# haliphinx/TCE-RVOS

Hardware: AMD Instinct MI355X
Metric: clips/s (T=5, 360×640, Swin-T) at 1/2/4/8 MI355X; mask IoU vs ref (higher is better)
Workload: dtype f32 (3xf16-split MFMA, f32 accumulate); 1 GPU; swin_t_p4w7 T=5 360x640 + 32-token text, B=1 clip per forward, flags --with_box_refine --binary --f_token 8 --qtrans (BASELINE config 2); clips_in_flight_per_gpu=1, clips_per_forward=1, same_clip_in_group=False, ranks_per_gpu=1, parallelism=clip-sharded x1

## Files before the change

include/tce_rvos.h:

```cpp
#ifndef TCE_RVOS_H
#define TCE_RVOS_H
#include <stdint.h>

#ifdef __cplusplus
extern "C" {
#endif

typedef void* tceStream;

int tce_abi_version(void);
const char* tce_last_error(void);

typedef struct {
  const float* A;
  const float* A2;
  const float* W;
  const float* bias;
  const float* res;
  float* C;
  int32_t M, N, K;
  int32_t lda, lda2, ldw, ldc, ldres;
  int32_t act, res_mode;
  int32_t batch;
  int64_t sA, sA2, sW, sBias, sC, sRes;
// ... 159 lines not shown
  float* out;
  const float *g_in, *be_in, *g_out, *be_out;
  int64_t ldx, lda2, ldres, ldo;
  int64_t sX, sA2, sRes, sOut;
  int32_t M, N, K, batch, a2_rows, act, res_mode;
  float eps_in, eps_out;
} tceRowLinArgs;
int64_t tce_rowlin_packed_bytes(int32_t N, int32_t K);
int tce_rowlin_pack_f32(const float* W, int64_t ldw, void* packed, int32_t N, int32_t K, tceStream stream);
int tce_rowlin_f32(const tceRowLinArgs* args, tceStream stream);

int64_t tce_conv3x3_packed_bytes(int32_t Cin, int32_t N);
int tce_conv3x3_pack_f32(const float* w, void* packed, int32_t Cin, int32_t N, tceStream stream);
int tce_conv3x3_f32(const float* x, int64_t ldx, const void* packed, const float* bias, float* out, int64_t ldo, int32_t T,
                    int32_t H, int32_t W, int32_t Cin, int32_t N, tceStream stream);

typedef struct {
  const float* x;
  const float* a2;
  const void* packed;
  const float* bo;
  const float* res;
  float* out;
  const float *g_out, *be_out;
  int64_t ldx, lda2, ldres, ldo;
  int64_t sX, sRes, sOut, sW;
  int32_t M, batch, a2_rows, res_mode, group;
  float eps_out;
  int32_t w_div;
} tceXattnArgs;
// ... 63 lines not shown
```

include/tce_rvos_debug.h:

```cpp
#ifndef TCE_RVOS_DEBUG_H
#define TCE_RVOS_DEBUG_H
#include <stdint.h>
#ifdef __cplusplus
extern "C" {
#endif
int tce_gemm_force_tile(int32_t tile);
int tce_debug_set_stamp_buffer(long long* dev_buf);
int tce_debug_set_epilogue(int32_t lds_staged);
int tce_debug_ffn_set_stamp_buffer(long long* dev_buf);
int tce_debug_ffn_set_half(int32_t mode);
int tce_debug_msda_set_lds(int32_t on);
int tce_debug_window_attn_set_mfma(int32_t on);
int tce_debug_mha_set_split(int32_t on);
int tce_debug_msda_set_fewq(int32_t on);
int tce_debug_conv3x3_set_waves(int32_t waves);
#ifdef __cplusplus
}
#endif
#endif
```

tce-rvos_amd/_lib.py:

```python
import ctypes as C
import os

HERE = os.path.dirname(os.path.abspath(__file__))
LIB_PATH = os.environ.get("TCE_LIB") or os.path.join(HERE, "lib", "libtce_rvos.so")

c_f = C.c_void_p
i32, i64, f32 = C.c_int32, C.c_int64, C.c_float


class GemmArgs(C.Structure):
    _fields_ = [("A", c_f), ("A2", c_f), ("W", c_f), ("bias", c_f), ("res", c_f), ("C", c_f),
                ("M", i32), ("N", i32), ("K", i32),
                ("lda", i32), ("lda2", i32), ("ldw", i32), ("ldc", i32), ("ldres", i32),
                ("act", i32), ("res_mode", i32), ("batch", i32),
                ("sA", i64), ("sA2", i64), ("sW", i64), ("sBias", i64), ("sC", i64), ("sRes", i64),
                ("conv", i32), ("T", i32), ("H", i32), ("Wd", i32), ("Cin", i32), ("Ho", i32), ("Wo", i32),
                ("kh", i32), ("kw", i32), ("stride", i32), ("pad", i32)]


class RowLinArgs(C.Structure):
    _fields_ = [("x", c_f), ("a2", c_f), ("packed", c_f), ("bias", c_f), ("res", c_f), ("out", c_f),
                ("g_in", c_f), ("be_in", c_f), ("g_out", c_f), ("be_out", c_f),
                ("ldx", i64), ("lda2", i64), ("ldres", i64), ("ldo", i64),
                ("sX", i64), ("sA2", i64), ("sRes", i64), ("sOut", i64),
# ... 93 lines not shown
    "tce_ffn_fused_split_f32": (i32, [c_f, i64, c_f, c_f, c_f, c_f, f32, c_f, c_f, f32, c_f, i64, i32, i32, i32, i32, c_f, i64, c_f, i32, c_f]),
    "tce_xattn_prepare_f32": (i32, [c_f, c_f, c_f, c_f, c_f, c_f, c_f, i32, i32, i32, c_f]),
    "tce_ffn_pack_batched_f32": (i32, [c_f, c_f, c_f, c_f, i32, i32, i32, c_f]),
    "tce_xattn_fused_f32": (i32, [C.POINTER(XattnArgs), c_f]),
    "tce_xattn_ffn_fused_f32": (i32, [C.POINTER(XattnArgs), C.POINTER(XattnFfnArgs), c_f]),
    "tce_ffn_pack_chain_f32": (i32, [c_f, c_f, c_f, c_f, i32, i32, c_f]),
    "tce_xattn_pack_f32": (i32, [c_f, c_f, c_f, c_f, c_f, i32, i32, i32, c_f]),
    "tce_xattn_prepare_lens_f32": (i32, [c_f, c_f, c_f, c_f, c_f, c_f, c_f, i32, i32, i32, c_f, c_f]),
    "tce_xattn_pack_lens_f32": (i32, [c_f, c_f, c_f, c_f, c_f, i32, i32, i32, c_f, c_f]),
    "tce_rowlin_packed_bytes": (i64, [i32, i32]),
    "tce_rowlin_pack_f32": (i32, [c_f, i64, c_f, i32, i32, c_f]),
    "tce_rowlin_f32": (i32, [C.POINTER(RowLinArgs), c_f]),
    "tce_conv3x3_packed_bytes": (i64, [i32, i32]),
    "tce_conv3x3_pack_f32": (i32, [c_f, c_f, i32, i32, c_f]),
    "tce_conv3x3_f32": (i32, [c_f, i64, c_f, c_f, c_f, i64, i32, i32, i32, i32, i32, c_f]),
    "tce_fewrow_linear_f32": (i32, [C.POINTER(FewRowArgs), c_f]),
    "tce_thin_linear_splits": (i32, [i32, i32, i32]),
    "tce_thin_partials_f32": (i32, [c_f, i64, i32, c_f, i32, c_f, i64, c_f, i32, i32, i32, c_f]),
    "tce_splitk_reduce_f32": (i32, [c_f, i32, i32, i32, c_f, i32, c_f, i32, i32, c_f, i32, c_f, c_f, f32, c_f]),
    "tce_mha_small64_splits_f32": (i32, [c_f, i32, c_f, c_f, i32, i32, f32, c_f]),
    "tce_swin_attn_packed_bytes": (i64, [i32]),
    "tce_swin_attn_pack_f32": (i32, [c_f, c_f, c_f, i32, c_f]),
    "tce_swin_attn_fused_f32": (i32, [c_f, i64, c_f, c_f, c_f, c_f, c_f, c_f, f32, c_f, i64, i32, i32, i32, i32, i32, c_f]),
    "tce_graph_begin": (i32, [c_f]),
    "tce_graph_end": (i32, [c_f, C.POINTER(C.c_void_p)]),
    "tce_graph_launch": (i32, [C.c_void_p, c_f]),
    "tce_graph_destroy": (i32, [C.c_void_p]),
    "tce_graph_group": (i32, [C.POINTER(C.c_void_p), i32, C.POINTER(C.c_void_p)]),
}

DEBUG_SIGNATURES = {
    "tce_gemm_force_tile": (i32, [i32]),
    "tce_debug_set_stamp_buffer": (i32, [c_f]),
    "tce_debug_set_epilogue": (i32, [i32]),
    "tce_debug_ffn_set_stamp_buffer": (i32, [c_f]),
    "tce_debug_ffn_set_half": (i32, [i32]),
    "tce_debug_msda_set_lds": (i32, [i32]),
    "tce_debug_window_attn_set_mfma": (i32, [i32]),
    "tce_debug_mha_set_split": (i32, [i32]),
    "tce_debug_msda_set_fewq": (i32, [i32]),
    "tce_debug_conv3x3_set_waves": (i32, [i32]),
}

_LIB = None


class TceError(RuntimeError):
    pass


def lib():
    global _LIB
    if _LIB is None:
        if not os.path.exists(LIB_PATH):
            raise TceError(f"{LIB_PATH} not found: build the HIP extension first "
                           f"(python -c 'import __graft_entry__ as g; g.build()'); there is no fallback path")
# ... 24 lines not shown
```

tce-rvos_amd/csrc/chain.hip:

```cpp
#include "common.h"
#include "gemm_epilogue.h"
#include "frag.h"
#include "../../include/tce_rvos.h"
#include "../../include/tce_rvos_debug.h"

namespace {

#ifndef FFN_ABL
#define FFN_ABL 0
#endif
static __device__ long long* g_ffn_stamps = nullptr;


template <int K, bool HAS_A2 = true>
__device__ __forceinline__ void load_x_frags(const float* __restrict__ x, const long long ldx,
                                             const float* __restrict__ a2, const long long lda2, const int a2_rows,
                                             const int m0, const int M, float* __restrict__ wt, const int lane,
                                             const float* __restrict__ g_in, const float* __restrict__ be_in,
                                             const float eps, h16x8 (&xh)[K / 16], h16x8 (&xl)[K / 16],
                                             const int single = 0) {
  constexpr int NP = K / 32;
  const int cr = lane >> 3, cp = (lane & 7) * 4;
  const int r = lane & 31, hf = lane >> 5;
  f32x4 v[NP][4];
// ... 834 lines not shown
      return;
    }
  }
  if (a.single) hipLaunchKernelGGL((rowlin_kernel<K, false, true>), grid, block, 0, s, a);
  else hipLaunchKernelGGL((rowlin_kernel<K, false, false>), grid, block, 0, s, a);
}

inline bool ffn_shape_ok(int C, int Hd) { return (C == 96 || C == 128 || C == 192 || C == 256) && Hd > 0 && Hd % 32 == 0; }
inline int ffn_waves(int C) { return C <= 128 ? 8 : 4; }
inline int ffn_pieces(int C) {
  const int w = ffn_waves(C);
  return (1 + 2 * (C / 16) + 4 * (C / 32) + w - 1) / w * w;
}
inline long long ffn_units(int C, int Hd) { return (long long)(Hd / 32 + 2) * ffn_pieces(C) * 64; }

struct FfnSplitPlan {
  int p = 0, k[2] = {0, 0}, nblk = 0;
  long long ws_floats = 0;
};
inline FfnSplitPlan ffn_split_plan(int M, int C, int Hd, int batch) {
  FfnSplitPlan best;
  const int B = tce_cdiv(M, 32 * ffn_waves(C)), NC = Hd / 32, CUS = 256;
  if (C != 256 || NC < 24 || batch < 1) return best;
  const int OVP = 3, OVF = 4;
  auto rounds = [&](long long wgs) { return (double)((wgs + CUS - 1) / CUS); };
  double best_cost = 0.75 * rounds((long long)B * batch) * (NC + 1 + OVP + OVF);
  for (int p = 1; p <= 2; ++p) {
    const int wd = p == 1 ? 0 : (p * NC - 2 * (1 + OVP)) / (p + 1), ws_ = p == 1 ? (NC + 1) / 2 : wd + 1 + OVP;
    int k[2] = {ws_, 0};
    bool ok = ws_ >= 1 && ws_ <= NC - 1;
    for (int i = 1; i < p && ok; ++i) {
      k[i] = wd - (NC - k[i - 1]);
      ok = k[i] >= 1 && k[i] <= NC - 1;
    }
    if (!ok) continue;
    const int busiest = ws_ > NC - k[p - 1] ? ws_ : NC - k[p - 1];
    const double cost = rounds((long long)tce_cdiv(B, p) * (p + 1) * batch) * (busiest + 1 + OVP + OVF);
// ... 11 lines not shown
}

static int g_ffn_half = 0;

template <int C, int WAVES>
void ffn_launch(const FfnArgs& a, int act, hipStream_t s, int batch = 1) {
  if constexpr (C == 256) {
    if (a.sp_p > 0 && act == 1) {
      const dim3 grid(tce_cdiv(a.nblk, a.sp_p) * (a.sp_p + 1), batch), block(64 * WAVES);
      if (a.single) hipLaunchKernelGGL((ffn_fused_kernel<C, WAVES, 1, true, 0, true>), grid, block, 0, s, a);
      else hipLaunchKernelGGL((ffn_fused_kernel<C, WAVES, 1, false, 0, true>), grid, block, 0, s, a);
      return;
    }
  }
  if constexpr (C <= 128 && WAVES == 8) {
    const long long b8 = (long long)tce_cdiv(a.M, 256) * batch, b4 = (long long)tce_cdiv(a.M, 128) * batch;
    const double c8 = (double)((b8 + 255) / 256);
    const long long rem = b4 % 512;
    const double c4 = (double)(b4 / 512) + (rem == 0 ? 0.0 : rem <= 256 ? 0.5 : 1.0);
    if (act == 2 && g_ffn_half >= 0 && (g_ffn_half > 0 || c4 <= c8)) {
      const dim3 grid(tce_cdiv(a.M, 128), batch), block(256);
      if (a.single) hipLaunchKernelGGL((ffn_fused_kernel<C, 4, 2, true>), grid, block, 0, s, a);
      else hipLaunchKernelGGL((ffn_fused_kernel<C, 4, 2, false>), grid, block, 0, s, a);
      return;
    }
  }
  const dim3 grid(tce_cdiv(a.M, 32 * WAVES), batch), block(64 * WAVES);
  if (a.single) {
    if (act == 1) hipLaunchKernelGGL((ffn_fused_kernel<C, WAVES, 1, true>), grid, block, 0, s, a);
    else if (act == 2) hipLaunchKernelGGL((ffn_fused_kernel<C, WAVES, 2, true>), grid, block, 0, s, a);
  } else {
    if (act == 1) hipLaunchKernelGGL((ffn_fused_kernel<C, WAVES, 1, false>), grid, block, 0, s, a);
    else if (act == 2) hipLaunchKernelGGL((ffn_fused_kernel<C, WAVES, 2, false>), grid, block, 0, s, a);
  }
// ... 128 lines not shown
  if (p_lo < P) stage_out[p_lo * 64 + lane] = ol;
}

constexpr int CONV_PAD_STAGES = 6;

struct ConvArgs {
  const float* x;
  const unsigned char* wpk;
  const float* bias;
  float* out;
  long long ldx, ldo;
  int H, W, M;
  int* range_flag;
  int single;
  int m_off;
};

#ifndef CONV_ABL
#define CONV_ABL 0
#endif

template <int BYTE_OFF>
__device__ __forceinline__ void gload16(f32x4& dst, const float* ptr) {
  asm volatile("global_load_dwordx4 %0, %1, off offset:%2" : "=v"(dst) : "v"(ptr), "n"(BYTE_OFF) : "memory");
}

template <int I, int N, typename F>
__device__ __forceinline__ void static_for(F&& f) {
  if constexpr (I < N) {
    f(std::integral_constant<int, I>{});
    static_for<I + 1, N>(f);
  }
}

template <int CIN, bool SINGLE, int WAVES = 4>
__global__ void __launch_bounds__(64 * WAVES, WAVES / 4) conv3x3_kernel(const ConvArgs p) {
  constexpr int NTL = 8;
  constexpr int PW = 16 / WAVES;
  constexpr int STAGE = 2 * NTL * PIECE;
  constexpr int R = 4;
  constexpr int XS = WAVES == 4 ? 6 : 4, LX = XS + 1;
  constexpr int NW = WAVES == 4 ? CONV_PAD_STAGES - 2 : 3, LW = NW + 2;
  constexpr int INFLIGHT = (2 + PW) * (LW - 3);
  static_assert(LW <= CONV_PAD_STAGES, "the packed stream's zero padding covers the weight lead");
  constexpr int BODY = 12;
  constexpr int ITERS = 3 * (CIN / 64);
  constexpr int KS = BODY * ITERS;
  static_assert(CIN % 64 == 0, "channel chunks come in groups of four");
  static_assert(BODY % R == 0 && BODY % XS == 0 && BODY % NW == 0 && LX >= LW, "ring positions are compile-time");
  static_assert(WAVES * WT_BYTES <= R * STAGE, "the epilogue's staging tiles alias the ring");
  __shared__ __attribute__((aligned(16))) unsigned char smem[R * STAGE];

  const int tid = threadIdx.x, lane = tid & 63;
  const int wave = __builtin_amdgcn_readfirstlane(tid >> 6);
  const int hf = lane >> 5;
  const int m0 = p.m_off + blockIdx.x * (32 * WAVES) + wave * 32;

  const int m = m0 + (lane & 31);
  const int px = m % p.W, py = (m / p.W) % p.H;
  const float* const zeros = reinterpret_cast<const float*>(p.wpk + (long long)(KS + CONV_PAD_STAGES) * STAGE) + 8 * hf;
  const float* const xme = p.x + (long long)min(m, p.M - 1) * p.ldx + 8 * hf;
  auto iter_ptrs = [&](const int it, const float* (&q)[3]) {
    const int dy = it / (CIN / 64) - 1, cq = it % (CIN / 64);
    const bool row_ok = it < ITERS && m < p.M && (unsigned)(py + dy) < (unsigned)p.H;
#pragma unroll
    for (int d = 0; d < 3; ++d) {
      const bool ok = row_ok && (unsigned)(px + d - 1) < (unsigned)p.W;
      q[d] = (ok ? xme + (long long)(dy * p.W + d - 1) * p.ldx : zeros) + 64 * cq;
    }
  };

  const float* wp = reinterpret_cast<const float*>(p.wpk + (long long)(PW * wave) * PIECE + lane * 16);
  unsigned char* const wdst = smem + (PW * wave) * PIECE + lane * 16;
  f32x4 wr[NW][PW];
  auto wload = [&](f32x4 (&dst)[PW]) {
    if (!(CONV_ABL & 8)) {
      gload16<0>(dst[0], wp);
      gload16<PIECE>(dst[1], wp);
      if constexpr (PW == 4) {
        gload16<2 * PIECE>(dst[2], wp);
        gload16<3 * PIECE>(dst[3], wp);
      }
    }
    wp += STAGE / 4;
  };
  auto wstore = [&](const f32x4 (&src)[PW], const int stage) {
#pragma unroll
    for (int q = 0; q < PW; ++q) *reinterpret_cast<f32x4*>(wdst + stage * STAGE + q * PIECE) = src[q];
  };

  f32x4 xr[XS][2];
  const float* cur[3];
  const float* nxt[3];
  iter_ptrs(0, cur);
  iter_ptrs(1, nxt);
  auto xload = [&](auto jjc, f32x4 (&dst)[2]) {
    constexpr int JJ = decltype(jjc)::value;
    constexpr int J = JJ % BODY;
    const float* const src = JJ < BODY ? cur[J % 3] : nxt[J % 3];
    if (CONV_ABL & 16) return;
    gload16<64 * (J / 3)>(dst[0], src);
    gload16<64 * (J / 3) + 16>(dst[1], src);
  };
  auto wait_loads = [&](auto nc, f32x4 (&xs)[2], f32x4 (&ws)[PW]) {
    constexpr int N = (CONV_ABL & 24) ? 0 : decltype(nc)::value;
    if constexpr (PW == 4) {
      asm volatile("s_waitcnt vmcnt(%6)"
                   : "+v"(xs[0]), "+v"(xs[1]), "+v"(ws[0]), "+v"(ws[1]), "+v"(ws[2]), "+v"(ws[3])
                   : "n"(N)
                   : "memory");
// ... 23 lines not shown
      }
    }
    if constexpr (m + LX >= 0) xload(std::integral_constant<int, m + LX>{}, xr[(m + LX) % XS]);
    if constexpr (m + LW >= 0) wload(wr[(m + LW) % NW]);
  });
  __syncthreads();
  h16x8 fh[4], fl[4];
  {
    const unsigned char* const st = smem + lane * 16;
    fh[0] = *reinterpret_cast<const h16x8*>(st);
    fl[0] = *reinterpret_cast<const h16x8*>(st + PIECE);
    fh[1] = *reinterpret_cast<const h16x8*>(st + 2 * PIECE);
    fl[1] = *reinterpret_cast<const h16x8*>(st + 3 * PIECE);
  }

  for (int it = 0; it < ITERS; ++it) {
    static_for<0, BODY>([&](auto jc) {
      constexpr int j = decltype(jc)::value;
      constexpr int nslot = (j + 1) % XS;
      const unsigned char* const st = smem + (j % R) * STAGE + lane * 16;
      unsigned nh[4], nl[4];
      auto tile = [&](auto tc) {
        constexpr int t = decltype(tc)::value;
#if CONV_ABL & 4
        const h16x8 k0 = fh[t % 4], k1 = fl[t % 4], k2 = bh, k3 = bl;
        asm volatile("" : : "v"(k0), "v"(k1), "v"(k2), "v"(k3));
#else
        if constexpr (!SINGLE) {
          acc[t] = __builtin_amdgcn_mfma_f32_32x32x16_f16(fh[t % 4], bl, acc[t], 0, 0, 0);
          acc[t] = __builtin_amdgcn_mfma_f32_32x32x16_f16(fl[t % 4], bh, acc[t], 0, 0, 0);
        }
// ... 36 lines not shown
      tile(std::integral_constant<int, 6>{});
      tile(std::integral_constant<int, 7>{});
      __builtin_amdgcn_sched_barrier(0);
      bh = __builtin_bit_cast(h16x8, u32x4{nh[0], nh[1], nh[2], nh[3]});
      bl = __builtin_bit_cast(h16x8, u32x4{nl[0], nl[1], nl[2], nl[3]});
    });
#pragma unroll
    for (int d = 0; d < 3; ++d) cur[d] = nxt[d];
    iter_ptrs(it + 2, nxt);
  }
  asm volatile("s_waitcnt vmcnt(0)" ::: "memory");
  __syncthreads();

  float* const wt = reinterpret_cast<float*>(smem + wave * WT_BYTES);
  tce_amax_t amax = 0;
  const ResTile none = {};
#pragma unroll
  for (int t = 0; t < NTL; ++t) {
    tile_bias_res<0>(acc[t], tile_bias_load(p.bias, 32 * t, lane), none, wt, lane);
    tile_store(acc[t], p.out, p.ldo, m0, p.M, 32 * t, wt, lane, amax);
  }
  tce_range_report(p.range_flag, amax);
}

__global__ void __launch_bounds__(256) conv3x3_pack_kernel(const float* __restrict__ w, unsigned char* __restrict__ out,
                                                           const int CIN, const long long units, const int single) {
  const long long u = (long long)blockIdx.x * 256 + threadIdx.x;
  if (u >= units) return;
  const int lane = (int)(u & 63);
  const long long pg = u >> 6;
  const int piece = (int)(pg & 15);
  const long long s = pg >> 4;
  const int r = lane & 31, hf = lane >> 5, t = piece >> 1;
  u32x4 o = {0u, 0u, 0u, 0u};
  if (s < 9 * CIN / 16) {
    const int it = (int)(s / 12), j = (int)(s % 12);
    const int dy = it / (CIN / 64), cc = 4 * (it % (CIN / 64)) + j / 3, dx = j % 3;
// ... 407 lines not shown
  TCE_CHECK_ARG(w && packed && tce_aligned16(packed), "tce_conv3x3_pack_f32: null / misaligned pointer");
  const long long units = conv3x3_units(Cin);
  hipLaunchKernelGGL(conv3x3_pack_kernel, dim3(tce_cdiv(units, 256)), dim3(256), 0, (hipStream_t)stream, w,
                     (unsigned char*)packed, Cin, units, tce_gemm_single_pass());
  TCE_CHECK_LAUNCH("tce_conv3x3_pack_f32");
  return TCE_OK;
}

static int g_conv3_waves = 0;
extern "C" int tce_debug_conv3x3_set_waves(int32_t waves) {
  TCE_CHECK_ARG(waves == 0 || waves == 4 || waves == 8, "tce_debug_conv3x3_set_waves: 0 (automatic), 4 or 8");
  g_conv3_waves = waves;
  return TCE_OK;
}

extern "C" int tce_conv3x3_f32(const float* x, int64_t ldx, const void* packed, const float* bias, float* out, int64_t ldo,
                               int32_t T, int32_t H, int32_t W, int32_t Cin, int32_t N, tceStream stream) {
  TCE_CHECK_ARG(conv3x3_shape_ok(Cin, N), "tce_conv3x3_f32: unsupported shape Cin=%d N=%d (256 -> 256)", Cin, N);
  TCE_CHECK_ARG(x && packed && out && T > 0 && H > 0 && W > 0 && (long long)T * H * W < (1ll << 31),
                "tce_conv3x3_f32: null pointer or bad sizes");
  TCE_CHECK_ARG(ldx >= Cin && ldx % 4 == 0 && ldo >= N && ldo % 4 == 0, "tce_conv3x3_f32: bad row pitch");
  TCE_CHECK_ARG(tce_aligned16(x) && tce_aligned16(out) && tce_aligned16(packed) && (!bias || tce_aligned16(bias)),
                "tce_conv3x3_f32: pointers must be 16-byte aligned");
  ConvArgs a;
  a.x = x; a.wpk = (const unsigned char*)packed; a.bias = bias; a.out = out;
  a.ldx = ldx; a.ldo = ldo; a.H = H; a.W = W; a.M = T * H * W;
  a.range_flag = tce_range_flag(); a.single = tce_gemm_single_pass();
  static const int env_force = []() { const char* e = getenv("TCE_CONV3_WAVES"); return e ? atoi(e) : 0; }();
  const int force = g_conv3_waves ? g_conv3_waves : env_force;
  const int r4 = tce_cdiv(tce_cdiv(a.M, 128), 256), r8 = tce_cdiv(tce_cdiv(a.M, 256), 256);
  a.m_off = 0;
  const int full8 = tce_cdiv(a.M, 256) / 256;
  const int rem_px = a.M - full8 * 256 * 256;
  const int mixed4 = 7 * full8 + 4 * tce_cdiv(tce_cdiv(rem_px, 128), 256);
  if (!force && !a.single && full8 >= 1 && rem_px > 0 && mixed4 < 4 * r4 && mixed4 < 7 * r8) {
    hipLaunchKernelGGL((conv3x3_kernel<256, false, 8>), dim3(full8 * 256), dim3(512), 0, (hipStream_t)stream, a);
    a.m_off = full8 * 256 * 256;
    hipLaunchKernelGGL((conv3x3_kernel<256, false>), dim3(tce_cdiv(rem_px, 128)), dim3(256), 0, (hipStream_t)stream, a);
    TCE_CHECK_LAUNCH("tce_conv3x3_f32(mixed)");
    return TCE_OK;
  }
  const int wide = force ? force : (4 * r4 > 7 * r8 ? 8 : 4);
  if (wide == 8 && !a.single) hipLaunchKernelGGL((conv3x3_kernel<256, false, 8>), dim3(tce_cdiv(a.M, 256)), dim3(512), 0, (hipStream_t)stream, a);
  else if (a.single) hipLaunchKernelGGL((conv3x3_kernel<256, true>), dim3(tce_cdiv(a.M, 128)), dim3(256), 0, (hipStream_t)stream, a);
  else hipLaunchKernelGGL((conv3x3_kernel<256, false>), dim3(tce_cdiv(a.M, 128)), dim3(256), 0, (hipStream_t)stream, a);
  TCE_CHECK_LAUNCH("tce_conv3x3_f32");
  return TCE_OK;
}

bool tce_patch_embed_mfma(const float* frames, const float* w, const float* b, const float* gamma, const float* beta,
                          float* out, int H, int W, int C, float eps, long long ntok, int Hp, int Wp, hipStream_t s) {
  if ((C != 96 && C != 128 && C != 192) || ntok >= (1ll << 31) || !tce_aligned16(frames) || !tce_aligned16(out) ||
      !tce_aligned16(w) || !tce_aligned16(b) || !tce_aligned16(gamma) || !tce_aligned16(beta))
    return false;
  const dim3 grid(tce_cdiv(ntok, 128)), block(256);
  int* const rf = tce_range_flag();
  const int single = tce_gemm_single_pass();
  if (C == 96) hipLaunchKernelGGL((patch_embed_mfma_kernel<3>), grid, block, 0, s, frames, w, b, gamma, beta, out, H, W, eps, (int)ntok, Hp, Wp, rf, single);
  else if (C == 128) hipLaunchKernelGGL((patch_embed_mfma_kernel<4>), grid, block, 0, s, frames, w, b, gamma, beta, out, H, W, eps, (int)ntok, Hp, Wp, rf, single);
  else hipLaunchKernelGGL((patch_embed_mfma_kernel<6>), grid, block, 0, s, frames, w, b, gamma, beta, out, H, W, eps, (int)ntok, Hp, Wp, rf, single);
  return true;
}
// ... 2 lines not shown
```

tce-rvos_amd/hazard.py:

```python
import contextlib
import traceback

import numpy as np
import torch

from . import _lib

F = 4


def strided(ptr, run_bytes, *dims):
    if not ptr or run_bytes <= 0 or any(c <= 0 for c, _ in dims):
        return np.zeros((0, 2), dtype=np.int64)
    starts = np.array([int(ptr)], dtype=np.int64)
    for count, stride in dims:
        if count == 1 or stride == 0:
            continue
        starts = (starts[:, None] + (np.arange(int(count), dtype=np.int64) * int(stride))[None, :]).reshape(-1)
    iv = np.stack([starts, starts + int(run_bytes)], 1)
    return merge(iv)


def dense(ptr, nbytes):
    return strided(ptr, int(nbytes))
# ... 325 lines not shown
         dense(_p(a[3]), 256 * 256 * F), dense(_p(a[10]), a[9] * 4)],
        [dense(_p(a[4]), a[9] * 8 * a[8] * 256 * F), dense(_p(a[5]), a[9] * 8 * a[8] * F), dense(_p(a[6]), a[9] * 8 * a[8] * 256 * F)]),
    "tce_xattn_pack_lens_f32": lambda a: (
        [dense(_p(a[0]), a[7] * a[5] * 256 * F), dense(_p(a[1]), a[7] * a[5] * 256 * F), dense(_p(a[2]), 257 * 256 * F), dense(_p(a[3]), 256 * 256 * F),
         dense(_p(a[8]), a[7] * 4)],
        [dense(_p(a[4]), a[7] * _lib.lib_raw().tce_ffn_packed_bytes(256, 8 * a[6]))]),
    "tce_rowlin_pack_f32": lambda a: ([strided(_p(a[0]), a[4] * F, (a[3], a[1] * F))],
                                      [dense(_p(a[2]), _lib.lib_raw().tce_rowlin_packed_bytes(a[3], a[4]))]),
    "tce_rowlin_f32": lambda a: _rowlin(_st(a[0])),
    "tce_conv3x3_pack_f32": lambda a: ([dense(_p(a[0]), a[3] * 9 * a[2] * F)],
                                       [dense(_p(a[1]), _lib.lib_raw().tce_conv3x3_packed_bytes(a[2], a[3]))]),
    "tce_conv3x3_f32": lambda a: (
        [strided(_p(a[0]), a[9] * F, (a[6] * a[7] * a[8], a[1] * F)), dense(_p(a[2]), _lib.lib_raw().tce_conv3x3_packed_bytes(a[9], a[10])),
         dense(_p(a[3]), a[10] * F)],
        [strided(_p(a[4]), a[10] * F, (a[6] * a[7] * a[8], a[5] * F))]),
    "tce_fewrow_linear_f32": lambda a: _fewrow(_st(a[0])),
    "tce_thin_partials_f32": lambda a: (
        [(strided(_p(a[0]), a[10] * F, (a[8], a[1] * F)) if a[2] == 0 else dense(_p(a[0]), a[2] * a[8] * a[10] * F)),
         dense(_p(a[3]), a[10] * F), strided(_p(a[5]), a[10] * F, (a[9], a[6] * F))],
        [dense(_p(a[7]), (a[10] // 256) * a[8] * a[9] * F)]),
    "tce_splitk_reduce_f32": lambda a: (
        [dense(_p(a[0]), a[1] * a[2] * a[3] * F), dense(_p(a[4]), a[3] * F), dense(_p(a[11]), a[3] * F), dense(_p(a[12]), a[3] * F)] +
        ([strided(_p(a[6]), a[3] * F, (a[2], a[7] * F))] if a[8] else []),
        [strided(_p(a[9]), a[3] * F, (a[2], a[10] * F))]),
    "tce_mha_small64_splits_f32": lambda a: ([dense(_p(a[0]), a[1] * a[4] * 3 * a[5] * 64 * F), dense(_p(a[2]), 3 * a[5] * 64 * F)],
                                             [dense(_p(a[3]), a[4] * a[5] * 64 * F)]),
    "tce_mha_small64_seqs_f32": lambda a: ([dense(_p(a[0]), a[1] * a[4] * a[5] * 3 * a[6] * 64 * F), dense(_p(a[2]), 3 * a[6] * 64 * F)],
                                           [dense(_p(a[3]), a[4] * a[5] * a[6] * 64 * F)]),
    "tce_mha_small64_lens_f32": lambda a: ([dense(_p(a[0]), a[1] * a[4] * a[5] * 3 * a[6] * 64 * F), dense(_p(a[2]), 3 * a[6] * 64 * F),
                                            dense(_p(a[8]), a[4] * 4)],
                                           [dense(_p(a[3]), a[4] * a[5] * a[6] * 64 * F)]),
    "tce_caption_lens_f32": lambda a: ([dense(_p(a[0]), a[1] * a[2] * 8)],
                                       [dense(_p(a[5]), a[1] * 4), dense(_p(a[6]), a[1] * a[2]), dense(_p(a[7]), a[1] * a[2] * a[4] * F)]),
    "tce_embed_ln_seqs_f32": lambda a: ([dense(_p(a[0]), a[7] * a[8] * 8), dense(_p(a[4]), a[9] * F), dense(_p(a[5]), a[9] * F)],
                                        [dense(_p(a[6]), a[7] * a[8] * a[9] * F)]),
    "tce_swin_attn_pack_f32": lambda a: ([dense(_p(a[0]), 3 * a[3] * a[3] * F), dense(_p(a[1]), a[3] * a[3] * F)],
                                         [dense(_p(a[2]), _lib.lib_raw().tce_swin_attn_packed_bytes(a[3]))]),
    "tce_swin_attn_fused_f32": lambda a: (
        [strided(_p(a[0]), a[14] * F, (a[11] * a[12] * a[13], a[1] * F)), dense(_p(a[2]), _lib.lib_raw().tce_swin_attn_packed_bytes(a[14])),
         dense(_p(a[3]), 3 * a[14] * F), dense(_p(a[4]), a[14] * F), dense(_p(a[5]), 169 * (a[14] // 32) * F),
         dense(_p(a[6]), a[14] * F), dense(_p(a[7]), a[14] * F)],
        [strided(_p(a[9]), a[14] * F, (a[11] * a[12] * a[13], a[10] * F))]),
}
NOT_LAUNCHES = {"tce_abi_version", "tce_last_error", "tce_gemm_select_tile", "tce_gemm_select_tile_ex", "tce_set_gemm_mode", "tce_set_gemm_mode_thread",
                "tce_get_gemm_mode", "tce_set_range_flag", "tce_groupnorm_nsplit", "tce_mha_ws_bytes", "tce_ffn_packed_bytes", "tce_ffn_split_ws_floats", "tce_ffn_split_counters",
                "tce_rowlin_packed_bytes", "tce_conv3x3_packed_bytes", "tce_swin_attn_packed_bytes", "tce_thin_linear_splits", "tce_graph_begin", "tce_graph_end", "tce_graph_launch",
                "tce_graph_destroy", "tce_graph_group"} | set(_lib.DEBUG_SIGNATURES)


class Launch:
    __slots__ = ("idx", "name", "stream", "tick", "clock", "reads", "writes", "site")

    def __repr__(self):
        return f"#{self.idx} {self.name} on stream {self.stream:#x} at {self.site}"


class Recorder:

    def __init__(self):
        self.launches = []
        self.clock = {}
# ... 168 lines not shown
```

tce-rvos_amd/model.py:

```python
import os
import types
import math
from collections import OrderedDict
from typing import List, Optional

import torch
from torch import nn

from . import ops
from .config import ModelConfig, config_from_args, index_buffers, param_shapes
from .weights import synth_tensor

ACT_RELU, ACT_GELU = ops.ACT_RELU, ops.ACT_GELU
RES_ADD, RES_MUL = ops.RES_ADD, ops.RES_MUL


class NestedTensor(object):

    def __init__(self, tensors, mask: Optional[torch.Tensor]):
        self.tensors = tensors
        self.mask = mask

    def to(self, device):
        nt = NestedTensor(self.tensors.to(device), self.mask.to(device) if self.mask is not None else None)
# ... 458 lines not shown
        return c

    def _text_pos(self, L, device):
        key = ("text_pos", L)
        tp = self._shape_cache.get(key)
        if tp is None:
            x = torch.arange(1, L + 1, dtype=torch.float32)
            x = x / (x[-1:] + 1e-6) * (2 * math.pi)
            dim_t = torch.arange(self.cfg.hidden_dim, dtype=torch.float32)
            dim_t = 10000.0 ** (2 * torch.div(dim_t, 2, rounding_mode="trunc") / self.cfg.hidden_dim)
            px = x[:, None] / dim_t
            tp = torch.stack((px[:, 0::2].sin(), px[:, 1::2].cos()), dim=2).flatten(1).to(device).contiguous()
            self._shape_cache[key] = tp
        return tp

    def _arena_bytes(self, T, H0, W0):
        tok0 = T * ((H0 + 3) // 4) * ((W0 + 3) // 4)
        return self.arena_bytes or int(tok0 * 4 * (2048 * 2.2 + 256 * 24) + (256 << 20))

    def _get_arena(self, T, H0, W0, device, slot=0):
        need = self._arena_bytes(T, H0, W0)
        ar = self._arenas.get(slot)
        if ar is None or ar.buf.numel() < need or ar.device != torch.device(device):
            ar = self._arenas[slot] = ops.Arena(device, need)
        return ar

    @torch.no_grad()
    def forward(self, samples, captions, targets, slot=0):
        if not isinstance(samples, NestedTensor) and not (hasattr(samples, "tensors") and hasattr(samples, "mask")):
            if len(samples) == 1:
                vids, mask = samples[0][None], None
            else:
                samples = nested_tensor_from_videos_list(samples)
# ... 254 lines not shown
        return run_clip(self, frames, text, img_h, img_w, arena, side_arena, side_stream, clone_outputs=False, valid=valid,
                        groups=groups, shared=shared, select=select,
                        fork2=(arena2, stream2) if os.environ.get("TCE_FORK2", "1") != "0" else None,
                        fork3=((arena3, stream3), (arena4, stream4)) if os.environ.get("TCE_FORK3", "1") != "0" else None)

    def _branch_resources(self, like, slot=0):
        T, _, H0, W0 = like.shape
        tok0 = T * ((H0 + 3) // 4) * ((W0 + 3) // 4)
        st = _side_streams(like.device, slot)
        return (ops.Arena(like.device, self._arena_bytes(T, H0, W0)),
                ops.Arena(like.device, T * self._tokens_per_frame(H0, W0) * 256 * 4 * 4 + (32 << 20)),
                st[0],
                ops.Arena(like.device, int(tok0 * 4 * (2048 * 1.1 + 256 * 4)) + (64 << 20)),
                st[1],
                ops.Arena(like.device, max(int(tok0 / 64 * 4 * (2048 + 256 * 12)) + int(tok0 / 16 * 4 * 256 * 8),
                                           int(tok0 / 4 * 4 * 256 * 5)) + (64 << 20)),
                st[2],
                ops.Arena(like.device, int(tok0 / 16 * 4 * (2048 * 1.1 + 256 * 12)) + (64 << 20)),
                st[3])

    @torch.no_grad()
    def hazard_check(self, frames, ids, img_hw=None, valid=None, slot=0, dry=False, groups=1, shared=False, ragged=False):
        from . import hazard
        frames = frames.to(torch.float32).contiguous()
        T, _, H0, W0 = frames.shape
        img_h, img_w = (float(H0), float(W0)) if img_hw is None else (float(img_hw[0]), float(img_hw[1]))
        self._ensure_packed()
        res = self._branch_resources(types.SimpleNamespace(shape=(T * (groups if shared else 1), 3, H0, W0), device=frames.device), slot)
        st = (frames.clone(), ids.to(frames.device).clone())
        run = lambda: self._run(st[0], self._group_text(st[1], ragged), img_h, img_w, res, valid=valid, shared=shared,
                                groups=groups)
# ... 202 lines not shown
```

tce-rvos_amd/ops.py:

```python
import ctypes as C

import os
import threading

import torch

from ._lib import GemmArgs, check, lib

ACT_NONE, ACT_RELU, ACT_GELU, ACT_RELU_AFTER_RES = 0, 1, 2, 3
RES_NONE, RES_ADD, RES_MUL = 0, 1, 2


class Arena:

    ALIGN = 256
    FLAGS = 1 << 14

    def __init__(self, device, nbytes):
        self.device = torch.device(device)
        self.buf = torch.empty(int(nbytes), dtype=torch.uint8, device=self.device)
        self.off = 0
        self.peak = 0
        self.flags = torch.zeros(self.FLAGS, dtype=torch.int32, device=self.device)
        self.flag_off = 0
# ... 962 lines not shown

    def go():
        check(lib().tce_rowlin_f32(C.byref(q), _stream()), "tce_rowlin_f32")
    if GEMM_PROFILE is None:
        go()
        return out
    e0, e1 = torch.cuda.Event(enable_timing=True), torch.cuda.Event(enable_timing=True)
    e0.record()
    go()
    e1.record()
    GEMM_PROFILE.append((f"rowlin_kernel<{K}", False, 2.0 * M * N * K * batch, e0, e1))
    return out


CONV3_MIN_PIXELS = int(os.environ.get("TCE_CONV3_MIN_PIXELS", 12000))


def conv3x3_pack(w_cl, Cin):
    _chk(w_cl, "w")
    N = w_cl.shape[0]
    nbytes = lib().tce_conv3x3_packed_bytes(Cin, N)
    if nbytes < 0 or w_cl.shape[1] != 9 * Cin or not w_cl.is_contiguous():
        raise ValueError(f"conv3x3_pack: unsupported shape N={N} Cin={Cin}")
    out = torch.empty(nbytes, dtype=torch.uint8, device=w_cl.device)
    check(lib().tce_conv3x3_pack_f32(w_cl.data_ptr(), out.data_ptr(), Cin, N, _stream()), "tce_conv3x3_pack_f32")
    return out


def conv3x3_register(w_cl, Cin, table=None):
    if lib().tce_conv3x3_packed_bytes(Cin, w_cl.shape[0]) < 0 or w_cl.shape[1] != 9 * Cin:
        return None
    r = _ROUTES if table is None else table
    key = (w_cl.data_ptr(), w_cl.shape[0], w_cl.shape[1], get_gemm_mode())
    if key not in r.conv3:
        r.conv3[key] = conv3x3_pack(w_cl, Cin)
        r.keep.append(w_cl)
    return r.conv3[key]


def conv3x3(x, pk, T, H, W, Cin, N, bias=None, out=None, alloc=None):
    _chk(x, "x")
    M = T * H * W
    if out is None:
        out = alloc(M, N) if alloc else torch.empty(M, N, dtype=torch.float32, device=x.device)

    def go():
        check(lib().tce_conv3x3_f32(x.data_ptr(), x.stride(0), pk.data_ptr(), bias.data_ptr() if bias is not None else None,
                                    out.data_ptr(), out.stride(0), T, H, W, Cin, N, _stream()), "tce_conv3x3_f32")
    if GEMM_PROFILE is None:
        go()
        return out
    e0, e1 = torch.cuda.Event(enable_timing=True), torch.cuda.Event(enable_timing=True)
    e0.record()
    go()
    e1.record()
    GEMM_PROFILE.append((f"conv3x3_kernel<{Cin}", True, 2.0 * M * N * 9 * Cin, e0, e1))
    return out


XATTN_MIN_ROWS = int(os.environ.get("TCE_XATTN_MIN_ROWS", 4000))
XATTN_PACK_FUSED = os.environ.get("TCE_XATTN_PACK_FUSED", "1") != "0"


# ... 114 lines not shown
```

Before: 161.7 clips/s.

## Split-K the 3x3 conv across pieces with a workspace reduction for small grids

```diff
diff --git a/include/tce_rvos.h b/include/tce_rvos.h
--- a/include/tce_rvos.h
+++ b/include/tce_rvos.h
@@ -197,6 +197,11 @@
 int tce_conv3x3_pack_f32(const float* w, void* packed, int32_t Cin, int32_t N, tceStream stream);
 int tce_conv3x3_f32(const float* x, int64_t ldx, const void* packed, const float* bias, float* out, int64_t ldo, int32_t T,
                     int32_t H, int32_t W, int32_t Cin, int32_t N, tceStream stream);
+int64_t tce_conv3x3_split_ws_floats(int32_t M, int32_t Cin, int32_t N);
+int32_t tce_conv3x3_split_pieces(int32_t M, int32_t Cin, int32_t N);
+int32_t tce_conv3x3_split_kstep(int32_t pieces, int32_t s);
+int tce_conv3x3_split_f32(const float* x, int64_t ldx, const void* packed, const float* bias, float* out, int64_t ldo, int32_t T,
+                          int32_t H, int32_t W, int32_t Cin, int32_t N, float* ws, int64_t ws_floats, tceStream stream);
 
 typedef struct {
   const float* x;
diff --git a/include/tce_rvos_debug.h b/include/tce_rvos_debug.h
--- a/include/tce_rvos_debug.h
+++ b/include/tce_rvos_debug.h
@@ -14,6 +14,7 @@
 int tce_debug_mha_set_split(int32_t on);
 int tce_debug_msda_set_fewq(int32_t on);
 int tce_debug_conv3x3_set_waves(int32_t waves);
+int tce_debug_conv3x3_set_pieces(int32_t pieces);
 #ifdef __cplusplus
 }
 #endif
diff --git a/tce-rvos_amd/_lib.py b/tce-rvos_amd/_lib.py
--- a/tce-rvos_amd/_lib.py
+++ b/tce-rvos_amd/_lib.py
@@ -131,6 +131,10 @@
     "tce_conv3x3_packed_bytes": (i64, [i32, i32]),
     "tce_conv3x3_pack_f32": (i32, [c_f, c_f, i32, i32, c_f]),
     "tce_conv3x3_f32": (i32, [c_f, i64, c_f, c_f, c_f, i64, i32, i32, i32, i32, i32, c_f]),
+    "tce_conv3x3_split_ws_floats": (i64, [i32, i32, i32]),
+    "tce_conv3x3_split_pieces": (i32, [i32, i32, i32]),
+    "tce_conv3x3_split_kstep": (i32, [i32, i32]),
+    "tce_conv3x3_split_f32": (i32, [c_f, i64, c_f, c_f, c_f, i64, i32, i32, i32, i32, i32, c_f, i64, c_f]),
     "tce_fewrow_linear_f32": (i32, [C.POINTER(FewRowArgs), c_f]),
     "tce_thin_linear_splits": (i32, [i32, i32, i32]),
     "tce_thin_partials_f32": (i32, [c_f, i64, i32, c_f, i32, c_f, i64, c_f, i32, i32, i32, c_f]),
@@ -157,6 +161,7 @@
     "tce_debug_mha_set_split": (i32, [i32]),
     "tce_debug_msda_set_fewq": (i32, [i32]),
     "tce_debug_conv3x3_set_waves": (i32, [i32]),
+    "tce_debug_conv3x3_set_pieces": (i32, [i32]),
 }
 
 _LIB = None
diff --git a/tce-rvos_amd/csrc/chain.hip b/tce-rvos_amd/csrc/chain.hip
--- a/tce-rvos_amd/csrc/chain.hip
+++ b/tce-rvos_amd/csrc/chain.hip
@@ -872,13 +872,31 @@
 }
 inline long long ffn_units(int C, int Hd) { return (long long)(Hd / 32 + 2) * ffn_pieces(C) * 64; }
 
+inline int tce_cu_count() {
+  static int cache[64] = {0};
+  int dev = 0;
+  if (hipGetDevice(&dev) != hipSuccess || dev < 0 || dev >= 64) {
+    (void)hipGetLastError();
+    return 256;
+  }
+  if (!cache[dev]) {
+    int n = 0;
+    if (hipDeviceGetAttribute(&n, hipDeviceAttributeMultiprocessorCount, dev) != hipSuccess || n <= 0) {
+      (void)hipGetLastError();
+      n = 256;
+    }
+    cache[dev] = n;
+  }
+  return cache[dev];
+}
+
 struct FfnSplitPlan {
   int p = 0, k[2] = {0, 0}, nblk = 0;
   long long ws_floats = 0;
 };
 inline FfnSplitPlan ffn_split_plan(int M, int C, int Hd, int batch) {
   FfnSplitPlan best;
-  const int B = tce_cdiv(M, 32 * ffn_waves(C)), NC = Hd / 32, CUS = 256;
+  const int B = tce_cdiv(M, 32 * ffn_waves(C)), NC = Hd / 32, CUS = tce_cu_count();
   if (C != 256 || NC < 24 || batch < 1) return best;
   const int OVP = 3, OVF = 4;
   auto rounds = [&](long long wgs) { return (double)((wgs + CUS - 1) / CUS); };
@@ -920,10 +938,10 @@
     }
   }
   if constexpr (C <= 128 && WAVES == 8) {
-    const long long b8 = (long long)tce_cdiv(a.M, 256) * batch, b4 = (long long)tce_cdiv(a.M, 128) * batch;
-    const double c8 = (double)((b8 + 255) / 256);
-    const long long rem = b4 % 512;
-    const double c4 = (double)(b4 / 512) + (rem == 0 ? 0.0 : rem <= 256 ? 0.5 : 1.0);
+    const long long b8 = (long long)tce_cdiv(a.M, 256) * batch, b4 = (long long)tce_cdiv(a.M, 128) * batch, cus = tce_cu_count();
+    const double c8 = (double)((b8 + cus - 1) / cus);
+    const long long rem = b4 % (2 * cus);
+    const double c4 = (double)(b4 / (2 * cus)) + (rem == 0 ? 0.0 : rem <= cus ? 0.5 : 1.0);
     if (act == 2 && g_ffn_half >= 0 && (g_ffn_half > 0 || c4 <= c8)) {
       const dim3 grid(tce_cdiv(a.M, 128), batch), block(256);
       if (a.single) hipLaunchKernelGGL((ffn_fused_kernel<C, 4, 2, true>), grid, block, 0, s, a);
@@ -1082,7 +1100,12 @@
   int* range_flag;
   int single;
   int m_off;
+  int nb, pieces;
+  float* ws;
 };
+
+constexpr int CONV_ITERS = 12;
+__host__ __device__ constexpr int conv3x3_piece_iter(const int pieces, const int s) { return s * CONV_ITERS / pieces; }
 
 #ifndef CONV_ABL
 #define CONV_ABL 0
@@ -1101,7 +1124,7 @@
   }
 }
 
-template <int CIN, bool SINGLE, int WAVES = 4>
+template <int CIN, bool SINGLE, int WAVES = 4, bool SPLIT = false>
 __global__ void __launch_bounds__(64 * WAVES, WAVES / 4) conv3x3_kernel(const ConvArgs p) {
   constexpr int NTL = 8;
   constexpr int PW = 16 / WAVES;
@@ -1117,12 +1140,17 @@
   static_assert(CIN % 64 == 0, "channel chunks come in groups of four");
   static_assert(BODY % R == 0 && BODY % XS == 0 && BODY % NW == 0 && LX >= LW, "ring positions are compile-time");
   static_assert(WAVES * WT_BYTES <= R * STAGE, "the epilogue's staging tiles alias the ring");
+  static_assert(!SPLIT || (ITERS == CONV_ITERS && WAVES == 4 && !SINGLE), "split pieces: CIN = 256, 128-pixel workgroups, split fp16");
   __shared__ __attribute__((aligned(16))) unsigned char smem[R * STAGE];
 
   const int tid = threadIdx.x, lane = tid & 63;
   const int wave = __builtin_amdgcn_readfirstlane(tid >> 6);
   const int hf = lane >> 5;
-  const int m0 = p.m_off + blockIdx.x * (32 * WAVES) + wave * 32;
+  const int blk = SPLIT ? (int)blockIdx.x % p.nb : (int)blockIdx.x;
+  const int piece = SPLIT ? (int)blockIdx.x / p.nb : 0;
+  const int i0 = SPLIT ? conv3x3_piece_iter(p.pieces, piece) : 0;
+  const int i1 = SPLIT ? conv3x3_piece_iter(p.pieces, piece + 1) : ITERS;
+  const int m0 = p.m_off + blk * (32 * WAVES) + wave * 32;
 
   const int m = m0 + (lane & 31);
   const int px = m % p.W, py = (m / p.W) % p.H;
@@ -1130,7 +1158,7 @@
   const float* const xme = p.x + (long long)min(m, p.M - 1) * p.ldx + 8 * hf;
   auto iter_ptrs = [&](const int it, const float* (&q)[3]) {
     const int dy = it / (CIN / 64) - 1, cq = it % (CIN / 64);
-    const bool row_ok = it < ITERS && m < p.M && (unsigned)(py + dy) < (unsigned)p.H;
+    const bool row_ok = it < i1 && m < p.M && (unsigned)(py + dy) < (unsigned)p.H;
 #pragma unroll
     for (int d = 0; d < 3; ++d) {
       const bool ok = row_ok && (unsigned)(px + d - 1) < (unsigned)p.W;
@@ -1138,7 +1166,7 @@
     }
   };
 
-  const float* wp = reinterpret_cast<const float*>(p.wpk + (long long)(PW * wave) * PIECE + lane * 16);
+  const float* wp = reinterpret_cast<const float*>(p.wpk + ((long long)i0 * BODY * STAGE) + (long long)(PW * wave) * PIECE + lane * 16);
   unsigned char* const wdst = smem + (PW * wave) * PIECE + lane * 16;
   f32x4 wr[NW][PW];
   auto wload = [&](f32x4 (&dst)[PW]) {
@@ -1160,8 +1188,8 @@
   f32x4 xr[XS][2];
   const float* cur[3];
   const float* nxt[3];
-  iter_ptrs(0, cur);
-  iter_ptrs(1, nxt);
+  iter_ptrs(i0, cur);
+  iter_ptrs(i0 + 1, nxt);
   auto xload = [&](auto jjc, f32x4 (&dst)[2]) {
     constexpr int JJ = decltype(jjc)::value;
     constexpr int J = JJ % BODY;
@@ -1215,7 +1243,7 @@
     fl[1] = *reinterpret_cast<const h16x8*>(st + 3 * PIECE);
   }
 
-  for (int it = 0; it < ITERS; ++it) {
+  for (int it = i0; it < i1; ++it) {
     static_for<0, BODY>([&](auto jc) {
       constexpr int j = decltype(jc)::value;
       constexpr int nslot = (j + 1) % XS;
@@ -1282,6 +1310,12 @@
 
   float* const wt = reinterpret_cast<float*>(smem + wave * WT_BYTES);
   tce_amax_t amax = 0;
+  if constexpr (SPLIT) {
+    float* const part = p.ws + (long long)piece * (p.M - p.m_off) * 256;
+#pragma unroll
+    for (int t = 0; t < NTL; ++t) tile_store(acc[t], part, 256, m0 - p.m_off, p.M - p.m_off, 32 * t, wt, lane, amax);
+    return;
+  }
   const ResTile none = {};
 #pragma unroll
   for (int t = 0; t < NTL; ++t) {
@@ -1289,6 +1323,23 @@
     tile_store(acc[t], p.out, p.ldo, m0, p.M, 32 * t, wt, lane, amax);
   }
   tce_range_report(p.range_flag, amax);
+}
+
+__global__ void __launch_bounds__(256) conv3x3_reduce_kernel(const float* __restrict__ ws, const int pieces, const int rows,
+                                                             const float* __restrict__ bias, float* __restrict__ out,
+                                                             const long long ldo, const int m_off, int* range_flag) {
+  const long long n4 = (long long)rows * 64, stride = (long long)gridDim.x * 256;
+  tce_amax_t amax = 0;
+  for (long long i = (long long)blockIdx.x * 256 + threadIdx.x; i < n4; i += stride) {
+    const f32x4* src = reinterpret_cast<const f32x4*>(ws) + i;
+    f32x4 v = src[0];
+    for (int s = 1; s < pieces; ++s) v += src[(long long)s * n4];
+    const int c4 = (int)(i & 63);
+    if (bias) v += reinterpret_cast<const f32x4*>(bias)[c4];
+    amax = tce_amax4(amax, v);
+    *reinterpret_cast<f32x4*>(out + (m_off + (i >> 6)) * ldo + 4 * c4) = v;
+  }
+  tce_range_report(range_flag, amax);
 }
 
 __global__ void __launch_bounds__(256) conv3x3_pack_kernel(const float* __restrict__ w, unsigned char* __restrict__ out,
@@ -1726,38 +1777,117 @@
   return TCE_OK;
 }
 
-extern "C" int tce_conv3x3_f32(const float* x, int64_t ldx, const void* packed, const float* bias, float* out, int64_t ldo,
-                               int32_t T, int32_t H, int32_t W, int32_t Cin, int32_t N, tceStream stream) {
-  TCE_CHECK_ARG(conv3x3_shape_ok(Cin, N), "tce_conv3x3_f32: unsupported shape Cin=%d N=%d (256 -> 256)", Cin, N);
+struct Conv3Plan {
+  int wide = 4;
+  int full8 = 0;
+  int m_narrow = 0;
+  int nb = 0;
+  int pieces = 1;
+  long long ws_floats = 0;
+};
+inline Conv3Plan conv3x3_plan(const int M, const int cus, const int single, const int force_waves, const int split, const int force_pieces) {
+  Conv3Plan pl;
+  const int r4 = tce_cdiv(tce_cdiv(M, 128), cus), r8 = tce_cdiv(tce_cdiv(M, 256), cus);
+  const int full8 = tce_cdiv(M, 256) / cus;
+  const int rem_px = M - full8 * 256 * cus;
+  const int mixed4 = 7 * full8 + 4 * tce_cdiv(tce_cdiv(rem_px, 128), cus);
+  if (!force_waves && !single && full8 >= 1 && rem_px > 0 && mixed4 < 4 * r4 && mixed4 < 7 * r8) {
+    pl.full8 = full8 * cus;
+    pl.m_narrow = full8 * 256 * cus;
+  } else {
+    pl.wide = force_waves ? force_waves : (4 * r4 > 7 * r8 ? 8 : 4);
+    if (single) pl.wide = 4;
+    if (pl.wide == 8) return pl;
+  }
+  pl.nb = tce_cdiv(M - pl.m_narrow, 128);
+  if (!split || single || pl.nb >= cus) return pl;
+  const double OVH = 0.5, LAUNCH = 0.3, RED_BPI = 8.0 * (3u << 20);
+  const long long px = M - pl.m_narrow;
+  auto cost = [&](int p) {
+    const double walk = (double)tce_cdiv((long long)pl.nb * p, cus) * (tce_cdiv(CONV_ITERS, p) + OVH);
+    return p == 1 ? walk : walk + LAUNCH + (double)(p + 1) * px * 1024.0 / RED_BPI;
+  };
+  int best = 1;
+  for (int p = 2; p <= 6; ++p)
+    if ((long long)pl.nb * p <= 2ll * cus && cost(p) < cost(best)) best = p;
+  if (force_pieces > 0) best = force_pieces;
+  if (best > 1) {
+    pl.pieces = best;
+    pl.ws_floats = (long long)best * px * 256;
+  }
+  return pl;
+}
+
+static int g_conv3_pieces = 0;
+extern "C" int tce_debug_conv3x3_set_pieces(int32_t pieces) {
+  TCE_CHECK_ARG(pieces >= 0 && pieces <= CONV_ITERS, "tce_debug_conv3x3_set_pieces: 0 (automatic) .. 12");
+  g_conv3_pieces = pieces;
+  return TCE_OK;
+}
+
+static int conv3_force_waves() {
+  static const int env_force = []() { const char* e = getenv("TCE_CONV3_WAVES"); return e ? atoi(e) : 0; }();
+  return g_conv3_waves ? g_conv3_waves : env_force;
+}
+
+static Conv3Plan conv3x3_plan_for(const int M, const bool split) {
+  return conv3x3_plan(M, tce_cu_count(), tce_gemm_single_pass(), conv3_force_waves(), split, g_conv3_pieces);
+}
+
+extern "C" int64_t tce_conv3x3_split_ws_floats(int32_t M, int32_t Cin, int32_t N) {
+  return conv3x3_shape_ok(Cin, N) && M > 0 ? conv3x3_plan_for(M, true).ws_floats : 0;
+}
+extern "C" int32_t tce_conv3x3_split_pieces(int32_t M, int32_t Cin, int32_t N) {
+  return conv3x3_shape_ok(Cin, N) && M > 0 ? conv3x3_plan_for(M, true).pieces : 0;
+}
+extern "C" int32_t tce_conv3x3_split_kstep(int32_t pieces, int32_t s) {
+  return pieces >= 1 && pieces <= CONV_ITERS && s >= 0 && s <= pieces ? 12 * conv3x3_piece_iter(pieces, s) : -1;
+}
+
+static int conv3x3_launch(const float* x, int64_t ldx, const void* packed, const float* bias, float* out, int64_t ldo, int32_t T,
+                          int32_t H, int32_t W, int32_t Cin, int32_t N, float* ws, int64_t ws_floats, const bool split, tceStream stream,
+                          const char* name) {
+  TCE_CHECK_ARG(conv3x3_shape_ok(Cin, N), "%s: unsupported shape Cin=%d N=%d (256 -> 256)", name, Cin, N);
   TCE_CHECK_ARG(x && packed && out && T > 0 && H > 0 && W > 0 && (long long)T * H * W < (1ll << 31),
-                "tce_conv3x3_f32: null pointer or bad sizes");
-  TCE_CHECK_ARG(ldx >= Cin && ldx % 4 == 0 && ldo >= N && ldo % 4 == 0, "tce_conv3x3_f32: bad row pitch");
+                "%s: null pointer or bad sizes", name);
+  TCE_CHECK_ARG(ldx >= Cin && ldx % 4 == 0 && ldo >= N && ldo % 4 == 0, "%s: bad row pitch", name);
   TCE_CHECK_ARG(tce_aligned16(x) && tce_aligned16(out) && tce_aligned16(packed) && (!bias || tce_aligned16(bias)),
-                "tce_conv3x3_f32: pointers must be 16-byte aligned");
+                "%s: pointers must be 16-byte aligned", name);
   ConvArgs a;
   a.x = x; a.wpk = (const unsigned char*)packed; a.bias = bias; a.out = out;
   a.ldx = ldx; a.ldo = ldo; a.H = H; a.W = W; a.M = T * H * W;
   a.range_flag = tce_range_flag(); a.single = tce_gemm_single_pass();
-  static const int env_force = []() { const char* e = getenv("TCE_CONV3_WAVES"); return e ? atoi(e) : 0; }();
-  const int force = g_conv3_waves ? g_conv3_waves : env_force;
-  const int r4 = tce_cdiv(tce_cdiv(a.M, 128), 256), r8 = tce_cdiv(tce_cdiv(a.M, 256), 256);
-  a.m_off = 0;
-  const int full8 = tce_cdiv(a.M, 256) / 256;
-  const int rem_px = a.M - full8 * 256 * 256;
-  const int mixed4 = 7 * full8 + 4 * tce_cdiv(tce_cdiv(rem_px, 128), 256);
-  if (!force && !a.single && full8 >= 1 && rem_px > 0 && mixed4 < 4 * r4 && mixed4 < 7 * r8) {
-    hipLaunchKernelGGL((conv3x3_kernel<256, false, 8>), dim3(full8 * 256), dim3(512), 0, (hipStream_t)stream, a);
-    a.m_off = full8 * 256 * 256;
-    hipLaunchKernelGGL((conv3x3_kernel<256, false>), dim3(tce_cdiv(rem_px, 128)), dim3(256), 0, (hipStream_t)stream, a);
-    TCE_CHECK_LAUNCH("tce_conv3x3_f32(mixed)");
-    return TCE_OK;
-  }
-  const int wide = force ? force : (4 * r4 > 7 * r8 ? 8 : 4);
-  if (wide == 8 && !a.single) hipLaunchKernelGGL((conv3x3_kernel<256, false, 8>), dim3(tce_cdiv(a.M, 256)), dim3(512), 0, (hipStream_t)stream, a);
-  else if (a.single) hipLaunchKernelGGL((conv3x3_kernel<256, true>), dim3(tce_cdiv(a.M, 128)), dim3(256), 0, (hipStream_t)stream, a);
-  else hipLaunchKernelGGL((conv3x3_kernel<256, false>), dim3(tce_cdiv(a.M, 128)), dim3(256), 0, (hipStream_t)stream, a);
-  TCE_CHECK_LAUNCH("tce_conv3x3_f32");
+  a.m_off = 0; a.nb = 0; a.pieces = 1; a.ws = nullptr;
+  hipStream_t s = (hipStream_t)stream;
+  const Conv3Plan pl = conv3x3_plan_for(a.M, split);
+  if (pl.pieces > 1)
+    TCE_CHECK_ARG(ws && tce_aligned16(ws) && ws_floats >= pl.ws_floats,
+                  "%s: workspace of %lld floats needed (tce_conv3x3_split_ws_floats), %lld given", name, pl.ws_floats, (long long)ws_floats);
+  if (pl.full8) hipLaunchKernelGGL((conv3x3_kernel<256, false, 8>), dim3(pl.full8), dim3(512), 0, s, a);
+  a.m_off = pl.m_narrow;
+  if (pl.wide == 8) hipLaunchKernelGGL((conv3x3_kernel<256, false, 8>), dim3(tce_cdiv(a.M, 256)), dim3(512), 0, s, a);
+  else if (a.single) hipLaunchKernelGGL((conv3x3_kernel<256, true>), dim3(pl.nb), dim3(256), 0, s, a);
+  else if (pl.pieces == 1) hipLaunchKernelGGL((conv3x3_kernel<256, false>), dim3(pl.nb), dim3(256), 0, s, a);
+  else {
+    a.nb = pl.nb; a.pieces = pl.pieces; a.ws = ws;
+    hipLaunchKernelGGL((conv3x3_kernel<256, false, 4, true>), dim3(pl.nb * pl.pieces), dim3(256), 0, s, a);
+    const int rows = a.M - a.m_off;
+    hipLaunchKernelGGL(conv3x3_reduce_kernel, dim3(std::min(tce_cdiv((long long)rows * 64, 256), 8 * tce_cu_count())), dim3(256), 0, s,
+                       (const float*)ws, pl.pieces, rows, bias, out, ldo, a.m_off, a.range_flag);
+  }
+  TCE_CHECK_LAUNCH(name);
   return TCE_OK;
+}
+
+extern "C" int tce_conv3x3_f32(const float* x, int64_t ldx, const void* packed, const float* bias, float* out, int64_t ldo,
+                               int32_t T, int32_t H, int32_t W, int32_t Cin, int32_t N, tceStream stream) {
+  return conv3x3_launch(x, ldx, packed, bias, out, ldo, T, H, W, Cin, N, nullptr, 0, false, stream, "tce_conv3x3_f32");
+}
+
+extern "C" int tce_conv3x3_split_f32(const float* x, int64_t ldx, const void* packed, const float* bias, float* out, int64_t ldo,
+                                     int32_t T, int32_t H, int32_t W, int32_t Cin, int32_t N, float* ws, int64_t ws_floats,
+                                     tceStream stream) {
+  return conv3x3_launch(x, ldx, packed, bias, out, ldo, T, H, W, Cin, N, ws, ws_floats, true, stream, "tce_conv3x3_split_f32");
 }
 
 bool tce_patch_embed_mfma(const float* frames, const float* w, const float* b, const float* gamma, const float* beta,
diff --git a/tce-rvos_amd/hazard.py b/tce-rvos_amd/hazard.py
--- a/tce-rvos_amd/hazard.py
+++ b/tce-rvos_amd/hazard.py
@@ -363,6 +363,11 @@
         [strided(_p(a[0]), a[9] * F, (a[6] * a[7] * a[8], a[1] * F)), dense(_p(a[2]), _lib.lib_raw().tce_conv3x3_packed_bytes(a[9], a[10])),
          dense(_p(a[3]), a[10] * F)],
         [strided(_p(a[4]), a[10] * F, (a[6] * a[7] * a[8], a[5] * F))]),
+    "tce_conv3x3_split_f32": lambda a: (
+        [strided(_p(a[0]), a[9] * F, (a[6] * a[7] * a[8], a[1] * F)), dense(_p(a[2]), _lib.lib_raw().tce_conv3x3_packed_bytes(a[9], a[10])),
+         dense(_p(a[3]), a[10] * F)],
+        [strided(_p(a[4]), a[10] * F, (a[6] * a[7] * a[8], a[5] * F)),
+         dense(_p(a[11]), _lib.lib_raw().tce_conv3x3_split_ws_floats(a[6] * a[7] * a[8], a[9], a[10]) * F)]),
     "tce_fewrow_linear_f32": lambda a: _fewrow(_st(a[0])),
     "tce_thin_partials_f32": lambda a: (
         [(strided(_p(a[0]), a[10] * F, (a[8], a[1] * F)) if a[2] == 0 else dense(_p(a[0]), a[2] * a[8] * a[10] * F)),
@@ -393,7 +398,8 @@
 }
 NOT_LAUNCHES = {"tce_abi_version", "tce_last_error", "tce_gemm_select_tile", "tce_gemm_select_tile_ex", "tce_set_gemm_mode", "tce_set_gemm_mode_thread",
                 "tce_get_gemm_mode", "tce_set_range_flag", "tce_groupnorm_nsplit", "tce_mha_ws_bytes", "tce_ffn_packed_bytes", "tce_ffn_split_ws_floats", "tce_ffn_split_counters",
-                "tce_rowlin_packed_bytes", "tce_conv3x3_packed_bytes", "tce_swin_attn_packed_bytes", "tce_thin_linear_splits", "tce_graph_begin", "tce_graph_end", "tce_graph_launch",
+                "tce_rowlin_packed_bytes", "tce_conv3x3_packed_bytes", "tce_conv3x3_split_ws_floats",
+                "tce_conv3x3_split_pieces", "tce_conv3x3_split_kstep", "tce_swin_attn_packed_bytes", "tce_thin_linear_splits", "tce_graph_begin", "tce_graph_end", "tce_graph_launch",
                 "tce_graph_destroy", "tce_graph_group"} | set(_lib.DEBUG_SIGNATURES)
 
 
diff --git a/tce-rvos_amd/model.py b/tce-rvos_amd/model.py
--- a/tce-rvos_amd/model.py
+++ b/tce-rvos_amd/model.py
@@ -496,9 +496,13 @@
             self._shape_cache[key] = tp
         return tp
 
+    @staticmethod
+    def _conv3_ws_bytes(T, H0, W0, strides):
+        return 4 * max(ops.conv3x3_split_ws_floats(T * (-(-H0 // s)) * (-(-W0 // s))) for s in strides)
+
     def _arena_bytes(self, T, H0, W0):
         tok0 = T * ((H0 + 3) // 4) * ((W0 + 3) // 4)
-        return self.arena_bytes or int(tok0 * 4 * (2048 * 2.2 + 256 * 24) + (256 << 20))
+        return self.arena_bytes or int(tok0 * 4 * (2048 * 2.2 + 256 * 24) + (256 << 20) + self._conv3_ws_bytes(T, H0, W0, (4, 8)))
 
     def _get_arena(self, T, H0, W0, device, slot=0):
         need = self._arena_bytes(T, H0, W0)
@@ -783,7 +787,7 @@
                 ops.Arena(like.device, int(tok0 * 4 * (2048 * 1.1 + 256 * 4)) + (64 << 20)),
                 st[1],
                 ops.Arena(like.device, max(int(tok0 / 64 * 4 * (2048 + 256 * 12)) + int(tok0 / 16 * 4 * 256 * 8),
-                                           int(tok0 / 4 * 4 * 256 * 5)) + (64 << 20)),
+                                           int(tok0 / 4 * 4 * 256 * 5)) + (64 << 20) + self._conv3_ws_bytes(T, H0, W0, (16, 32))),
                 st[2],
                 ops.Arena(like.device, int(tok0 / 16 * 4 * (2048 * 1.1 + 256 * 12)) + (64 << 20)),
                 st[3])
diff --git a/tce-rvos_amd/ops.py b/tce-rvos_amd/ops.py
--- a/tce-rvos_amd/ops.py
+++ b/tce-rvos_amd/ops.py
@@ -1000,6 +1000,11 @@
 
 
 CONV3_MIN_PIXELS = int(os.environ.get("TCE_CONV3_MIN_PIXELS", 12000))
+CONV3_SPLIT = os.environ.get("TCE_CONV3_SPLIT", "1") != "0"
+
+
+def conv3x3_split_ws_floats(M, Cin=256, N=256):
+    return int(lib().tce_conv3x3_split_ws_floats(M, Cin, N)) if CONV3_SPLIT else 0
 
 
 def conv3x3_pack(w_cl, Cin):
@@ -1030,9 +1035,17 @@
     if out is None:
         out = alloc(M, N) if alloc else torch.empty(M, N, dtype=torch.float32, device=x.device)
 
+    nws = conv3x3_split_ws_floats(M, Cin, N) if alloc else 0
+    ws = alloc(nws) if nws else None
+
     def go():
-        check(lib().tce_conv3x3_f32(x.data_ptr(), x.stride(0), pk.data_ptr(), bias.data_ptr() if bias is not None else None,
-                                    out.data_ptr(), out.stride(0), T, H, W, Cin, N, _stream()), "tce_conv3x3_f32")
+        bp = bias.data_ptr() if bias is not None else None
+        if ws is not None:
+            check(lib().tce_conv3x3_split_f32(x.data_ptr(), x.stride(0), pk.data_ptr(), bp, out.data_ptr(), out.stride(0), T, H, W,
+                                              Cin, N, ws.data_ptr(), nws, _stream()), "tce_conv3x3_split_f32")
+        else:
+            check(lib().tce_conv3x3_f32(x.data_ptr(), x.stride(0), pk.data_ptr(), bp, out.data_ptr(), out.stride(0), T, H, W, Cin,
+                                        N, _stream()), "tce_conv3x3_f32")
     if GEMM_PROFILE is None:
         go()
         return out
```

Measured after the change: 164.5 clips/s, median of 6. 1.7% higher.
